# king159/Pair-Net

Hardware: AMD Instinct MI355X
Metric: images/sec (whole node), 100-query 800x1333, 1/2/4/8 MI355X (higher is better)
Workload: dtype f32

## Files before the change

### include/pairnet_hip.h

```cpp
#ifndef PAIRNET_HIP_H_
#define PAIRNET_HIP_H_

#include <stdint.h>

#ifdef __cplusplus
extern "C" {
#endif

#define PN_ABI_VERSION 34
int pn_abi_version(void);

#define PN_GEMM_RELU       1
#define PN_GEMM_A_COLMAJOR 2
#define PN_GEMM_FORCE_TILE 4
#define PN_GEMM_FORCE_SKINNY 8
#define PN_GEMM_FORCE_TILE64 16
#define PN_GEMM_FORCE_TILE128x64 32
#define PN_GEMM_RELU_AFTER_RES 128
#define PN_GEMM_GELU 256
#define PN_GEMM_RESERVE_SHIFT 16
#define PN_GEMM_RESERVE(n) ((((n) / 8) & 0x3ff) << PN_GEMM_RESERVE_SHIFT)
#define PN_GEMM_KSPLIT_SHIFT 26
#define PN_GEMM_KSPLIT(n) (((n) & 31) << PN_GEMM_KSPLIT_SHIFT)

// ... 442 lines not shown
typedef struct pn_gemm_s3_desc {
  const void* A;  const void* A2;  int32_t a2_from_col;
  const void* W;  const float* bias;
  int32_t M, N, K;
  int32_t relu;
  float* C;       int64_t ldc;
  void* CS;
  void* CS_pos;   const float* pos;  int32_t pos_rows;
  const void* res_s3;  const float* gamma;  const float* beta;  float eps;
  int32_t flags;
  int32_t act;  const float* res;  int64_t ldres;
} pn_gemm_s3_desc;
#define PN_GEMM_S3_TILE96 1
#define PN_GEMM_S3_TILE192 2
int pn_gemm_s3_f32(const pn_gemm_s3_desc* d, void* stream);

int pn_uniform_f32(float* out, int64_t n, int nsites, uint32_t site_stride, uint64_t seed,
                   uint32_t rank, uint32_t step, uint32_t site, void* stream);
int pn_seg_targets(const int64_t* table, const int32_t* row_ind, const int32_t* col_ind,
                   const int32_t* lsa_status, int nlsa, const int64_t* gt_labels, int64_t gt_len,
                   int64_t out_len, int L, int B, int Q, int C, int64_t Mtot, int64_t* labels,
                   int64_t* matched, int32_t* mcount, int32_t* status, void* stream);
int pn_uncertain_points_f32(const float* maps, int64_t nmaps, const int64_t* matched, int64_t M,
                            int B, int Q, int h, int w, const float* cand, const float* tail, int S,
                            int k, int Np, uint32_t* keys, float* pts, void* stream);
int pn_point_sample_rows_f32(const void* maps, int maps_are_u8, int64_t nmaps, const int64_t* idx,
                             const float* pts, float* out, int64_t M, int h, int w, int Np,
                             void* stream);
int pn_mask_point_loss_f32(const float* x, const float* t, const int64_t* matched, int64_t M, int Np,
                           int L, int Ml, float w_mask, float w_dice, float dice_eps,
// ... 80 lines not shown
```

### pair-net_amd/csrc/gemm_s3.hip

```cpp
#include "common.h"
#include "s3_common.h"

__device__ __forceinline__ void s3_glds16(const void* g, void* l) {
  __builtin_amdgcn_global_load_lds((const __attribute__((address_space(1))) void*)g,
                                   (__attribute__((address_space(3))) void*)l, 16, 0, 0);
}

__device__ __forceinline__ int64_t pos8_offset(int row, int col, int N) {
  return ((((int64_t)(row >> 5) * (N >> 4) + (col >> 4)) * 2 + ((col >> 3) & 1)) * 32 + (row & 31)) * 8;
}

__global__ __launch_bounds__(256) void k_s3_split(const float* __restrict__ X, int64_t ld,
                                                  const float* __restrict__ add, int add_rows,
                                                  uint4* __restrict__ S, int R, int K) {
  const int KB = K >> 4;
  const int lane = threadIdx.x & 63;
  const int64_t piece = (int64_t)blockIdx.x * 4 + (threadIdx.x >> 6);
  const int64_t npieces = (int64_t)((R + 31) >> 5) * KB;
  if (piece >= npieces) return;
  const int rb = (int)(piece / KB), kb = (int)(piece - (int64_t)rb * KB);
  const int r = rb * 32 + (lane & 31), k = kb * 16 + (lane >> 5) * 8;
  float v[8];
  if (r < R) {
    const float4 a = ld4(X + (int64_t)r * ld + k), b = ld4(X + (int64_t)r * ld + k + 4);
// ... 74 lines not shown
    }
    if (p.relu == 3) {
#pragma unroll
      for (int i = 0; i < 8; ++i) v[i] = fmaxf(v[i], 0.f);
    }
    if (p.C && row < p.M) {
      float* c = p.C + (int64_t)row * p.ldc + n0 + 16 * j + 8 * lh;
      st4(c, make_float4(v[0], v[1], v[2], v[3]));
      st4(c + 4, make_float4(v[4], v[5], v[6], v[7]));
    }
    if (p.CS) {
      s3_frag q0, q1, q2;
      s3_split8(v, q0, q1, q2);
      uint4* o = p.CS + ((int64_t)rb * KBo + (n0 >> 4) + j) * 192 + lane;
      o[0] = q0.u; o[64] = q1.u; o[128] = q2.u;
    }
  }
}

#ifndef S3_LATE_B
#define S3_LATE_B 0
#endif
template <bool LN>
__global__ __launch_bounds__(512, 1) void k_gemm_s3(const s3_args p) {
  constexpr int MB = 3, LATE_B = S3_LATE_B;
  constexpr int AH = 9 * 64, AST = 2 * AH;
  constexpr int BH = 24 * 64, BST = 2 * BH;
  constexpr int BRING = 3 * AST;
  __shared__ __attribute__((aligned(1024))) uint4 smem[3 * AST + 2 * BST];
  const int tid = threadIdx.x, lane = tid & 63, wave = __builtin_amdgcn_readfirstlane(tid >> 6);
// ... 129 lines not shown
      mma(s + 2 < S ? s + 2 : -1);
      if (s + 1 < S) drain_bar();
      as = as == 2 ? 0 : as + 1;
    }
  }

  const int n0 = tn * 256 + wave * 32;
  if (!LN) {
    if (n0 < N) {
#pragma unroll
      for (int m = 0; m < MB; ++m)
        if (rb0 + m < RB) s3_block_epilogue(acc[m], p, rb0 + m, n0, lane);
    }
    return;
  }
  const int li = lane & 31, lh = lane >> 5;
  const bool cols_ok = n0 < N;
  float v[MB][2][8];
#pragma unroll
  for (int m = 0; m < MB; ++m)
#pragma unroll
    for (int j = 0; j < 2; ++j)
#pragma unroll
      for (int i = 0; i < 4; ++i) {
        const auto sw = __builtin_amdgcn_permlane32_swap(__float_as_uint(acc[m][8 * j + i]),
                                                         __float_as_uint(acc[m][8 * j + 4 + i]), false, false);
        v[m][j][i] = __uint_as_float(sw[0]);
        v[m][j][4 + i] = __uint_as_float(sw[1]);
      }
  if (p.bias && cols_ok) {
#pragma unroll
    for (int j = 0; j < 2; ++j) {
      const float4 b0 = ld4(p.bias + n0 + 16 * j + 8 * lh), b1 = ld4(p.bias + n0 + 16 * j + 8 * lh + 4);
      const float bb[8] = {b0.x, b0.y, b0.z, b0.w, b1.x, b1.y, b1.z, b1.w};
#pragma unroll
      for (int m = 0; m < MB; ++m)
#pragma unroll
        for (int i = 0; i < 8; ++i) v[m][j][i] += bb[i];
    }
  }
  if (p.relu) {
#pragma unroll
    for (int m = 0; m < MB; ++m)
#pragma unroll
      for (int j = 0; j < 2; ++j)
#pragma unroll
        for (int i = 0; i < 8; ++i) v[m][j][i] = fmaxf(v[m][j][i], 0.f);
  }
  if (LN) {
#pragma clang fp contract(off)
    if (p.RES) {
#pragma unroll
      for (int m = 0; m < MB; ++m)
#pragma unroll
        for (int j = 0; j < 2; ++j) {
          const uint4* in = p.RES + ((int64_t)min(rb0 + m, RB - 1) * 16 + wave * 2 + j) * 192 + lane;
          s3_frag q0, q1, q2;
          q0.u = in[0]; q1.u = in[64]; q2.u = in[128];
          float r[8];
          s3_join8(q0, q1, q2, r);
#pragma unroll
          for (int i = 0; i < 8; ++i) v[m][j][i] += r[i];
        }
    }
    float* red = (float*)smem;
    __syncthreads();
    float s1[MB];
#pragma unroll
    for (int m = 0; m < MB; ++m) {
      float s = 0.f;
#pragma unroll
      for (int j = 0; j < 2; ++j)
#pragma unroll
        for (int i = 0; i < 8; ++i) s += v[m][j][i];
      s += __shfl_xor(s, 32, 64);
      if (lh == 0) red[wave * 96 + m * 32 + li] = s;
    }
    __syncthreads();
#pragma unroll
    for (int m = 0; m < MB; ++m) {
      float s = 0.f;
#pragma unroll
      for (int w = 0; w < 8; ++w) s += red[w * 96 + m * 32 + li];
      s1[m] = s * (1.f / 256.f);
    }
#pragma unroll
    for (int m = 0; m < MB; ++m) {
      float s = 0.f;
#pragma unroll
      for (int j = 0; j < 2; ++j)
#pragma unroll
        for (int i = 0; i < 8; ++i) { v[m][j][i] -= s1[m]; s += v[m][j][i] * v[m][j][i]; }
      s += __shfl_xor(s, 32, 64);
      if (lh == 0) red[768 + wave * 96 + m * 32 + li] = s;
    }
    __syncthreads();
    float g[2][8], be[2][8];
#pragma unroll
    for (int j = 0; j < 2; ++j) {
      const float4 g0 = ld4(p.gamma + n0 + 16 * j + 8 * lh), g1 = ld4(p.gamma + n0 + 16 * j + 8 * lh + 4);
      const float4 e0 = ld4(p.beta + n0 + 16 * j + 8 * lh), e1 = ld4(p.beta + n0 + 16 * j + 8 * lh + 4);
      g[j][0] = g0.x; g[j][1] = g0.y; g[j][2] = g0.z; g[j][3] = g0.w; g[j][4] = g1.x; g[j][5] = g1.y; g[j][6] = g1.z; g[j][7] = g1.w;
      be[j][0] = e0.x; be[j][1] = e0.y; be[j][2] = e0.z; be[j][3] = e0.w; be[j][4] = e1.x; be[j][5] = e1.y; be[j][6] = e1.z; be[j][7] = e1.w;
    }
#pragma unroll
    for (int m = 0; m < MB; ++m) {
      float s = 0.f;
#pragma unroll
      for (int w = 0; w < 8; ++w) s += red[768 + w * 96 + m * 32 + li];
      const float rstd = 1.f / sqrtf(s * (1.f / 256.f) + p.eps);
#pragma unroll
      for (int j = 0; j < 2; ++j)
#pragma unroll
        for (int i = 0; i < 8; ++i) v[m][j][i] = (v[m][j][i] * rstd) * g[j][i] + be[j][i];
    }
  }
  if (!cols_ok) return;
  const int KBo = p.nout >> 4;
#pragma unroll
  for (int m = 0; m < MB; ++m) {
    if (rb0 + m >= RB) break;
    const int row = (rb0 + m) * 32 + li;
#pragma unroll
    for (int j = 0; j < 2; ++j) {
      if (p.C && row < M) {
        float* c = p.C + (int64_t)row * p.ldc + n0 + 16 * j + 8 * lh;
        st4(c, make_float4(v[m][j][0], v[m][j][1], v[m][j][2], v[m][j][3]));
        st4(c + 4, make_float4(v[m][j][4], v[m][j][5], v[m][j][6], v[m][j][7]));
      }
      const int64_t piece = ((int64_t)(rb0 + m) * KBo + (n0 >> 4) + j) * 192 + lane;
      if (p.CS) {
        s3_frag q0, q1, q2;
        s3_split8(v[m][j], q0, q1, q2);
        uint4* o = p.CS + piece;
        o[0] = q0.u; o[64] = q1.u; o[128] = q2.u;
      }
      if (p.CSP) {
        const float* pp = p.pos + pos8_offset(min(row, M - 1) % p.pos_rows, n0 + 16 * j + 8 * lh, p.nout);
        const float4 p0 = ld4(pp), p1 = ld4(pp + 4);
        const float w[8] = {v[m][j][0] + p0.x, v[m][j][1] + p0.y, v[m][j][2] + p0.z, v[m][j][3] + p0.w,
                            v[m][j][4] + p1.x, v[m][j][5] + p1.y, v[m][j][6] + p1.z, v[m][j][7] + p1.w};
        s3_frag q0, q1, q2;
        s3_split8(w, q0, q1, q2);
        uint4* o = p.CSP + piece;
        o[0] = q0.u; o[64] = q1.u; o[128] = q2.u;
      }
    }
  }
}

__global__ __launch_bounds__(512, 1) void k_gemm_s3_wide(const s3_args p) {
  constexpr int MB = 3;
  constexpr int AS = 9 * 64, WS = 24 * 64;
  constexpr int WRING = 4 * AS;
  __shared__ __attribute__((aligned(1024))) uint4 smem[4 * AS + 3 * WS];
  const int tid = threadIdx.x, lane = tid & 63, wave = __builtin_amdgcn_readfirstlane(tid >> 6);
  const int grp = wave >> 2, wq = wave & 3;
  const int KB = p.K >> 4;
  const int RB = (p.M + 31) >> 5, CB = (p.N + 31) >> 5;
  const int nt = (p.N + 255) >> 8, mt = (RB + 2 * MB - 1) / (2 * MB);
  const int t = xcd_tile_index(blockIdx.x, nt * mt);
  const int tm = t / nt, tn = t - tm * nt;
  const int rb0 = tm * 2 * MB + grp * MB;
// ... 98 lines not shown
      if (j + 1 < KB) drain_bar();
      ws = ws == 2 ? 0 : ws + 1;
    }
  }
#pragma unroll
  for (int m = 0; m < MB; ++m) {
    if (rb0 + m >= RB) break;
#pragma unroll
    for (int c = 0; c < 2; ++c) {
      const int n0 = tn * 256 + wq * 64 + c * 32;
      if (n0 < p.N) s3_block_epilogue(acc[m][c], p, rb0 + m, n0, lane);
    }
  }
}

__global__ __launch_bounds__(256) void k_gemm_s3_narrow(const s3_args p, const int col0) {
  const int lane = threadIdx.x & 63;
  const int KB = p.K >> 4, RB = (p.M + 31) >> 5, ncb = (p.N - col0) >> 5;
  const int unit = blockIdx.x * 4 + (threadIdx.x >> 6);
  if (unit >= RB * ncb) return;
  const int rb = unit / ncb, cb = (col0 >> 5) + unit - rb * ncb;
  const uint4* ga = ((p.A2 && (cb >> 3) >= p.a2_from_tile) ? p.A2 : p.A) + (int64_t)rb * KB * 192 + lane;
  const uint4* gw = p.W + (int64_t)cb * KB * 192 + lane;
  f32x16 acc;
#pragma unroll
  for (int r = 0; r < 16; ++r) acc[r] = 0.f;
  constexpr int PA[6] = {2, 1, 0, 1, 0, 0}, PB[6] = {0, 1, 2, 0, 1, 0};
  constexpr int D = 4;
  s3_frag a[D][3], b[D][3];
  auto load = [&](int kb, int slot) {
// ... 22 lines not shown

extern "C" int pn_s3_split_f32(const float* X, int64_t ld, const float* add, int add_rows, void* S,
                               int rows, int K, void* stream) {
  if (!X || !S || rows <= 0 || K <= 0 || K % 16 || ld % 4 || (add && add_rows <= 0)) return PN_BAD_ARG;
  const int64_t np = (int64_t)((rows + 31) / 32) * (K / 16);
  k_s3_split<<<dim3((unsigned)((np + 3) / 4)), dim3(256), 0, (hipStream_t)stream>>>(
      X, ld, add, add ? add_rows : 1, (uint4*)S, rows, K);
  return PN_LAUNCH_CHECK();
}

extern "C" int pn_s3_join_f32(const void* S, float* X, int64_t ld, int rows, int K, void* stream) {
  if (!X || !S || rows <= 0 || K <= 0 || K % 16 || ld % 4) return PN_BAD_ARG;
  const int64_t np = (int64_t)((rows + 31) / 32) * (K / 16);
  k_s3_join<<<dim3((unsigned)((np + 3) / 4)), dim3(256), 0, (hipStream_t)stream>>>(
      (const uint4*)S, X, ld, rows, K);
  return PN_LAUNCH_CHECK();
}

extern "C" int pn_gemm_s3_f32(const pn_gemm_s3_desc* d, void* stream) {
  if (!d || !d->A || !d->W || d->M <= 0 || d->N <= 0 || d->K <= 0) return PN_BAD_ARG;
  if (d->K % 32 || d->N % 32) return PN_BAD_ARG;
  if (!d->C && !d->CS && !d->CS_pos) return PN_BAD_ARG;
  if (d->C && (d->ldc % 4 || d->ldc < d->N)) return PN_BAD_ARG;
  if (d->A2 && (d->a2_from_col <= 0 || d->a2_from_col % 256)) return PN_BAD_ARG;
  if (d->CS_pos && (!d->pos || d->pos_rows <= 0)) return PN_BAD_ARG;
  const bool ln = d->gamma != nullptr;
  if (ln && (d->N != 256 || !d->beta || d->relu)) return PN_BAD_ARG;
  if (!ln && d->res_s3) return PN_BAD_ARG;
  if (d->res && (ln || d->ldres % 4 || d->ldres < d->N)) return PN_BAD_ARG;
  if (d->act < 0 || d->act > 3 || (ln && d->act)) return PN_BAD_ARG;
// ... 47 lines not shown
```

### pair-net_amd/head.py

```python
import math
from collections import OrderedDict

import torch

from . import hip
from . import plans
from .plans import Arena, PlanCache, measure_bytes
from .config import ConfigDict

INSTANCE_OFFSET = 1000


def _decoder_param_shapes(prefix, num_layers, ffn_dim, out):
    for i in range(num_layers):
        p = "%s.layers.%d." % (prefix, i)
        for a in (0, 1):
            out[p + "attentions.%d.attn.in_proj_weight" % a] = (768, 256)
            out[p + "attentions.%d.attn.in_proj_bias" % a] = (768,)
            out[p + "attentions.%d.attn.out_proj.weight" % a] = (256, 256)
            out[p + "attentions.%d.attn.out_proj.bias" % a] = (256,)
        out[p + "ffns.0.layers.0.0.weight"] = (ffn_dim, 256)
        out[p + "ffns.0.layers.0.0.bias"] = (ffn_dim,)
        out[p + "ffns.0.layers.1.weight"] = (256, ffn_dim)
        out[p + "ffns.0.layers.1.bias"] = (256,)
# ... 87 lines not shown
        self.device = None
        self.w = None
        self._plans = PlanCache()
        self._arenas, self._post_arenas, self._consts, self._pe = {}, {}, {}, OrderedDict()
        self._dummies = {}
        self._post = OrderedDict()
        self._pan_jobs = []
        self.graph_after = 1
        self.exact_mask_order = True
        self.conv_algo = "winograd4"
        self.use_graphs = False
        self.grid_reserve = 0
        self.fuse_ppn_front = True
        self.fuse_mask_pack = True
        self.gather_mask_stencil = True
        self.fuse_lateral_upadd = False
        self.enc_fused_ln = ("proj", "ffn")
        self.group_input_convs = False
        self.gemm_arithmetic = "bf16x3"
        self.msda_s3_out = False
        self.fused_pair_masks = True
        self.init_weights()

    def param_shapes(self):
        s = OrderedDict()
        Q, R = self.num_obj_query, self.num_rel_query
        _decoder_param_shapes("relation_decoder", self.num_rel_layers, self.rel_ffn, s)
        s["rel_query_embed.weight"] = (R, 256)
        s["rel_query_embed2.weight"] = (2 * R, 256)
        s["rel_query_embed3.weight"] = (2 * R, 256)
# ... 499 lines not shown
            if "ffn" in self.enc_fused_ln:
                hip.linear_res_ln(pl.H, w[p + "ffns.0.layers.1.weight"],
                                  w[p + "ffns.0.layers.1.bias"], X12, w[p + "norms.1.weight"],
                                  w[p + "norms.1.bias"], X2)
            else:
                hip.linear(pl.H, w[p + "ffns.0.layers.1.weight"], w[p + "ffns.0.layers.1.bias"],
                           Y2, res=X12)
                hip.layernorm(Y2, w[p + "norms.1.weight"], w[p + "norms.1.bias"], X2)

    def _encoder_s3(self, pl):
        w, B, SN = self.w, pl.B, pl.SN
        pd = "pixel_decoder."
        M, F = B * SN, self.enc_ffn
        X2 = pl.X.view(-1, 256)
        pos8 = (pl.enc_pos8, SN)
        hip.s3_split(X2, pl.XS)
        hip.s3_split(X2, pl.XPS, add=pl.enc_pos)
        for i in range(self.num_enc_layers):
            p = pd + "encoder.layers.%d." % i
            a = p + "attentions.0."
            last = i + 1 == self.num_enc_layers
            hip.gemm_s3(pl.XS, w[a + "voa.weight.s3"], M, 544, 256, bias=w[a + "voa.bias"],
                        out=pl.VOA.view(-1, 544), a2=pl.XPS, a2_from_col=256)
            if self.msda_s3_out:
                hip.msda(pl.VOA, 544, pl.VOA.view(-1)[256:], 544, pl.SS, B, pl.shapes, s3_out=True)
            else:
                hip.msda(pl.VOA, 544, pl.VOA.view(-1)[256:], 544, pl.S, B, pl.shapes)
                hip.s3_split(pl.S.view(-1, 256), pl.SS)
            hip.gemm_s3(pl.SS, w[a + "output_proj.weight.s3"], M, 256, 256,
                        bias=w[a + "output_proj.bias"], out_s3=pl.X1S, res_s3=pl.XS,
                        gamma=w[p + "norms.0.weight"], beta=w[p + "norms.0.bias"])
            hip.gemm_s3(pl.X1S, w[p + "ffns.0.layers.0.0.weight.s3"], M, F, 256,
                        bias=w[p + "ffns.0.layers.0.0.bias"], relu=True, out_s3=pl.HS)
            hip.gemm_s3(pl.HS, w[p + "ffns.0.layers.1.weight.s3"], M, 256, F,
                        bias=w[p + "ffns.0.layers.1.bias"], res_s3=pl.X1S,
                        gamma=w[p + "norms.1.weight"], beta=w[p + "norms.1.bias"],
                        out=X2 if last else None, out_s3=None if last else pl.XS,
                        out_s3_pos=None if last else pl.XPS, pos=pos8)

    def _mlp3(self, prefix, src, dst, pl):
        w = self.w
        hip.linear(src, w[prefix + ".0.weight"], w[prefix + ".0.bias"], pl.m1, relu=True)
        hip.linear(pl.m1, w[prefix + ".2.weight"], w[prefix + ".2.bias"], pl.m2, relu=True)
        hip.linear(pl.m2, w[prefix + ".4.weight"], w[prefix + ".4.bias"], dst)

    def _mask_logits(self, me, pl, out):
        Q = self.num_obj_query
        hip.gemm(me, pl.MF, out, M=Q, N=pl.HW2, K=256, lda=256, ldw=256, ldc=pl.HW2,
                 batch=pl.B, sA=Q * 256, sW=pl.HW2 * 256, sC=Q * pl.HW2)

    def _head_embed(self, q, pl, with_cls, full_mask, cls_out=None, mp_out=None, normed=False):
        w, B, Q = self.w, pl.B, self.num_obj_query
        cls_out = pl.cls if cls_out is None else cls_out
# ... 207 lines not shown
        for f, c in zip(feats, self.in_channels):
            if not f.is_cuda or f.dtype != torch.float32 or f.shape[1] != c or not (nchw or nhwc):
                raise RuntimeError("feats must be fp32 [B,C,H,W] device tensors with channels %s, "
                                   "all contiguous or all in channels_last memory format"
                                   % self.in_channels)
        if self.device is None:
            self.to(feats[0].device)
        shapes = [tuple(feats[3 - l].shape[-2:]) for l in range(3)]
        self._feats_nhwc = nhwc
        return B, shapes, tuple(feats[0].shape[-2:])

    def _run_stage(self, which, pl, feats=None):
        cfg = (self.exact_mask_order, self.conv_algo, self.fuse_ppn_front, self.grid_reserve,
               tuple(self.enc_fused_ln), self.group_input_convs,
               getattr(self, "fuse_mask_pack", True), self.gemm_arithmetic, self.msda_s3_out,
               self._fused_pair_masks(),
               getattr(self, "gather_mask_stencil", True), getattr(self, "fuse_lateral_upadd", False))
        if pl.graph_cfg != cfg:
            pl.graph_a = pl.graph_b = None
            pl.graphs_a = OrderedDict()
            pl.graph_c = PlanCache(self.POST_VIEWS)
            pl.graph_cfg = cfg
        cur = torch.cuda.current_stream(self.device)
        pl.streams[cur.cuda_stream] = cur
        try:
            self._run_stage_on(which, pl, feats, cur)
        finally:
            plans.note_use(cur)

    def _run_stage_on(self, which, pl, feats, cur):
        if which == "a":
# ... 349 lines not shown
```

### pair-net_amd/hip.py

```python
import contextlib
import ctypes as C
import os
import threading

import torch

from .build import LIB_PATH

LIB_PATH = os.environ.get("PAIRNET_LIB") or LIB_PATH

_i32, _i64, _f32, _vp = C.c_int32, C.c_int64, C.c_float, C.c_void_p

GEMM_RELU, GEMM_A_COLMAJOR, GEMM_FORCE_TILE, GEMM_FORCE_SKINNY = 1, 2, 4, 8
GEMM_GELU = 256
GEMM_FORCE_TILE64, GEMM_FORCE_TILE128x64 = 16, 32
GEMM_RELU_AFTER_RES = 128
GEMM_GROUP_MAX = 18


class GemmDesc(C.Structure):
    _fields_ = [("A", _vp), ("lda", _i64), ("strideA", _i64),
                ("Aadd", _vp), ("ldaadd", _i64), ("aadd_rows", _i32),
                ("aadd_from_col", _i32),
                ("W", _vp), ("ldw", _i64), ("strideW", _i64),
# ... 4 lines not shown
                ("flags", _i32),
                ("splitk_scratch", _vp), ("splitk_scratch_floats", _i64)]


class GemmS3Desc(C.Structure):
    _fields_ = [("A", _vp), ("A2", _vp), ("a2_from_col", _i32),
                ("W", _vp), ("bias", _vp),
                ("M", _i32), ("N", _i32), ("K", _i32), ("relu", _i32),
                ("C", _vp), ("ldc", _i64),
                ("CS", _vp),
                ("CS_pos", _vp), ("pos", _vp), ("pos_rows", _i32),
                ("res_s3", _vp), ("gamma", _vp), ("beta", _vp), ("eps", _f32), ("flags", _i32),
                ("act", _i32), ("res", _vp), ("ldres", _i64)]


_SIGS = {
    "pn_abi_version": (C.c_int, []),
    "pn_s3_bytes": (_i64, [_i32, _i32]),
    "pn_s3_split_f32": (C.c_int, [_vp, _i64, _vp, _i32, _vp, _i32, _i32, _vp]),
    "pn_s3_join_f32": (C.c_int, [_vp, _vp, _i64, _i32, _i32, _vp]),
    "pn_gemm_s3_f32": (C.c_int, [C.POINTER(GemmS3Desc), _vp]),
    "pn_gemm_f32": (C.c_int, [C.POINTER(GemmDesc), _vp]),
    "pn_gemm_variant": (C.c_int, [C.POINTER(GemmDesc)]),
    "pn_gemm_grid_size": (C.c_int, [C.POINTER(GemmDesc)]),
    "pn_gemm_wgs_per_cu": (C.c_int, []),
    "pn_gemm_group_f32": (C.c_int, [C.POINTER(GemmDesc), C.c_int, _vp]),
    "pn_conv2d_nhwc_f32": (C.c_int, [_vp, _vp, _vp, _vp] + [_i32] * 10 + [_vp]),
    "pn_conv2d_nhwc_ex_f32": (C.c_int, [_vp] * 5 + [_i32] * 10 + [_vp, _i64, _vp]),
    "pn_bottleneck_proj_f32": (C.c_int, [_vp] * 8 + [_i32] * 8 + [_vp, _i64, _vp]),
    "pn_stem7x7s2_f32": (C.c_int, [_vp, _vp, _vp, _vp, _i32, _i32, _i32, _i32, _vp]),
    "pn_maxpool3x3s2_nhwc_f32": (C.c_int, [_vp, _vp, _i32, _i32, _i32, _i32, _vp]),
    "pn_winograd_f23_input_f32": (C.c_int, [_vp, _vp, _i32, _i32, _i32, _i32, _vp]),
    "pn_winograd_f23_output_f32": (C.c_int, [_vp, _vp, _vp, _i32, _i32, _i32, _i32, _i32, _vp]),
    "pn_winograd_f43_input_f32": (C.c_int, [_vp, _vp, _i32, _i32, _i32, _i32, _vp]),
    "pn_winograd_f43_output_f32": (C.c_int, [_vp, _vp, _vp, _i32, _i32, _i32, _i32, _i32, _vp]),
    "pn_layernorm_f32": (C.c_int, [_vp, _vp, _vp, _vp, _i64, _i32, _f32, _vp]),
# ... 605 lines not shown
        d.pos, d.pos_rows = _ptr(pos), pr
    d.res_s3, d.gamma, d.beta, d.eps = _ptr(res_s3), _ptr(gamma), _ptr(beta), eps
    d.flags = (1 if tile96 else 0) | (2 if tile192 else 0)
    d.act = 3 if relu_after else 2 if gelu else 0
    if res is not None:
        Mr, ldr = _rowmajor(res)
        assert Mr == M and res.shape[1] >= N
        d.res, d.ldres = _ptr(res), ldr
    nbytes = 6.0 * (M * K + N * K) + (4.0 * M * N if out is not None else 0.0) + \
        6.0 * M * N * ((out_s3 is not None) + (out_s3_pos is not None) + (res_s3 is not None))
    name = "k_gemm_s3<ln>" if gamma is not None else "k_gemm_s3"
    _check(_launch(name, 2.0 * M * N * K, nbytes, lambda: lib().pn_gemm_s3_f32(C.byref(d), _stream()),
                   meta=(M, N, K, 1, False)), "pn_gemm_s3_f32")


def layernorm_rows(x, gamma, beta, out, eps=1e-5):
    rows, ldx = _rowmajor(x)
    ro, ldo = _rowmajor(out)
    assert ro == rows and out.shape[1] == x.shape[1]
    _check(_launch("k_ln_rows", 0.0, 8.0 * rows * x.shape[1],
                   lambda: lib().pn_layernorm_rows_f32(_ptr(x), ldx, _ptr(gamma), _ptr(beta),
                                                       _ptr(out), ldo, rows, x.shape[1], eps,
                                                       _stream())), "pn_layernorm_rows_f32")


def layernorm_rows_s3(x, gamma, beta, out_s3, eps=1e-5):
    rows, ldx = _rowmajor(x)
    Cc = x.shape[1]
    assert out_s3.numel() >= s3_floats(rows, Cc)
    _check(_launch("k_ln_rows<s3>", 0.0, 10.0 * rows * Cc,
# ... 1319 lines not shown
```

Before: 229.4.

## Fuse encoder FFN into one kernel keeping hidden activations on-chip

Adds a k_gemm_s3_ffn kernel that computes the encoder FFN (GEMM1 + bias + ReLU, then GEMM2 + bias + residual + LayerNorm) in a single launch. The hidden activation is produced in 256-wide chunks, split into s3 pieces and written straight into shared memory for the second GEMM. This avoids writing and re-reading the large hidden tensor HS through global memory, and saves one launch per layer. The LN epilogue is factored into a shared helper. In exchange, each workgroup recomputes over the whole F dimension with a fixed 3-row-block tile and a complex wave-specialised schedule, so parallelism is limited to M/96 workgroups, which risks underfilling the GPU.

```diff
diff --git a/include/pairnet_hip.h b/include/pairnet_hip.h
--- a/include/pairnet_hip.h
+++ b/include/pairnet_hip.h
@@ -480,6 +480,17 @@
 #define PN_GEMM_S3_TILE96 1
 #define PN_GEMM_S3_TILE192 2
 int pn_gemm_s3_f32(const pn_gemm_s3_desc* d, void* stream);
+typedef struct pn_gemm_s3_ffn_desc {
+  const void* X;  const void* W1;  const float* b1;
+  const void* W2; const float* b2;
+  int32_t M, N, K, F;
+  int32_t act;
+  float* C;       int64_t ldc;
+  void* CS;
+  void* CS_pos;   const float* pos;  int32_t pos_rows;
+  const void* res_s3;  const float* gamma;  const float* beta;  float eps;
+} pn_gemm_s3_ffn_desc;
+int pn_gemm_s3_ffn_f32(const pn_gemm_s3_ffn_desc* d, void* stream);
 
 int pn_uniform_f32(float* out, int64_t n, int nsites, uint32_t site_stride, uint64_t seed,
                    uint32_t rank, uint32_t step, uint32_t site, void* stream);
diff --git a/pair-net_amd/csrc/gemm_s3.hip b/pair-net_amd/csrc/gemm_s3.hip
--- a/pair-net_amd/csrc/gemm_s3.hip
+++ b/pair-net_amd/csrc/gemm_s3.hip
@@ -112,6 +112,145 @@
       s3_split8(v, q0, q1, q2);
       uint4* o = p.CS + ((int64_t)rb * KBo + (n0 >> 4) + j) * 192 + lane;
       o[0] = q0.u; o[64] = q1.u; o[128] = q2.u;
+    }
+  }
+}
+
+__device__ __forceinline__ void s3_ln_epilogue(const f32x16 (&acc)[3], const s3_args& p, uint4* smem,
+                                               int rb0, int n0, int wave, int lane) {
+  constexpr int MB = 3;
+  const int M = p.M, RB = (M + 31) >> 5;
+  const int li = lane & 31, lh = lane >> 5;
+  const bool cols_ok = n0 < p.N;
+  float v[MB][2][8];
+#pragma unroll
+  for (int m = 0; m < MB; ++m)
+#pragma unroll
+    for (int j = 0; j < 2; ++j)
+#pragma unroll
+      for (int i = 0; i < 4; ++i) {
+        const auto sw = __builtin_amdgcn_permlane32_swap(__float_as_uint(acc[m][8 * j + i]),
+                                                         __float_as_uint(acc[m][8 * j + 4 + i]), false, false);
+        v[m][j][i] = __uint_as_float(sw[0]);
+        v[m][j][4 + i] = __uint_as_float(sw[1]);
+      }
+  if (p.bias && cols_ok) {
+#pragma unroll
+    for (int j = 0; j < 2; ++j) {
+      const float4 b0 = ld4(p.bias + n0 + 16 * j + 8 * lh), b1 = ld4(p.bias + n0 + 16 * j + 8 * lh + 4);
+      const float bb[8] = {b0.x, b0.y, b0.z, b0.w, b1.x, b1.y, b1.z, b1.w};
+#pragma unroll
+      for (int m = 0; m < MB; ++m)
+#pragma unroll
+        for (int i = 0; i < 8; ++i) v[m][j][i] += bb[i];
+    }
+  }
+  if (p.relu) {
+#pragma unroll
+    for (int m = 0; m < MB; ++m)
+#pragma unroll
+      for (int j = 0; j < 2; ++j)
+#pragma unroll
+        for (int i = 0; i < 8; ++i) v[m][j][i] = fmaxf(v[m][j][i], 0.f);
+  }
+  {
+#pragma clang fp contract(off)
+    if (p.RES) {
+#pragma unroll
+      for (int m = 0; m < MB; ++m)
+#pragma unroll
+        for (int j = 0; j < 2; ++j) {
+          const uint4* in = p.RES + ((int64_t)min(rb0 + m, RB - 1) * 16 + wave * 2 + j) * 192 + lane;
+          s3_frag q0, q1, q2;
+          q0.u = in[0]; q1.u = in[64]; q2.u = in[128];
+          float r[8];
+          s3_join8(q0, q1, q2, r);
+#pragma unroll
+          for (int i = 0; i < 8; ++i) v[m][j][i] += r[i];
+        }
+    }
+    float* red = (float*)smem;
+    __syncthreads();
+    float s1[MB];
+#pragma unroll
+    for (int m = 0; m < MB; ++m) {
+      float s = 0.f;
+#pragma unroll
+      for (int j = 0; j < 2; ++j)
+#pragma unroll
+        for (int i = 0; i < 8; ++i) s += v[m][j][i];
+      s += __shfl_xor(s, 32, 64);
+      if (lh == 0) red[wave * 96 + m * 32 + li] = s;
+    }
+    __syncthreads();
+#pragma unroll
+    for (int m = 0; m < MB; ++m) {
+      float s = 0.f;
+#pragma unroll
+      for (int w = 0; w < 8; ++w) s += red[w * 96 + m * 32 + li];
+      s1[m] = s * (1.f / 256.f);
+    }
+#pragma unroll
+    for (int m = 0; m < MB; ++m) {
+      float s = 0.f;
+#pragma unroll
+      for (int j = 0; j < 2; ++j)
+#pragma unroll
+        for (int i = 0; i < 8; ++i) { v[m][j][i] -= s1[m]; s += v[m][j][i] * v[m][j][i]; }
+      s += __shfl_xor(s, 32, 64);
+      if (lh == 0) red[768 + wave * 96 + m * 32 + li] = s;
+    }
+    __syncthreads();
+    float g[2][8], be[2][8];
+#pragma unroll
+    for (int j = 0; j < 2; ++j) {
+      const float4 g0 = ld4(p.gamma + n0 + 16 * j + 8 * lh), g1 = ld4(p.gamma + n0 + 16 * j + 8 * lh + 4);
+      const float4 e0 = ld4(p.beta + n0 + 16 * j + 8 * lh), e1 = ld4(p.beta + n0 + 16 * j + 8 * lh + 4);
+      g[j][0] = g0.x; g[j][1] = g0.y; g[j][2] = g0.z; g[j][3] = g0.w; g[j][4] = g1.x; g[j][5] = g1.y; g[j][6] = g1.z; g[j][7] = g1.w;
+      be[j][0] = e0.x; be[j][1] = e0.y; be[j][2] = e0.z; be[j][3] = e0.w; be[j][4] = e1.x; be[j][5] = e1.y; be[j][6] = e1.z; be[j][7] = e1.w;
+    }
+#pragma unroll
+    for (int m = 0; m < MB; ++m) {
+      float s = 0.f;
+#pragma unroll
+      for (int w = 0; w < 8; ++w) s += red[768 + w * 96 + m * 32 + li];
+      const float rstd = 1.f / sqrtf(s * (1.f / 256.f) + p.eps);
+#pragma unroll
+      for (int j = 0; j < 2; ++j)
+#pragma unroll
+        for (int i = 0; i < 8; ++i) v[m][j][i] = (v[m][j][i] * rstd) * g[j][i] + be[j][i];
+    }
+  }
+  if (!cols_ok) return;
+  const int KBo = p.nout >> 4;
+#pragma unroll
+  for (int m = 0; m < MB; ++m) {
+    if (rb0 + m >= RB) break;
+    const int row = (rb0 + m) * 32 + li;
+#pragma unroll
+    for (int j = 0; j < 2; ++j) {
+      if (p.C && row < M) {
+        float* c = p.C + (int64_t)row * p.ldc + n0 + 16 * j + 8 * lh;
+        st4(c, make_float4(v[m][j][0], v[m][j][1], v[m][j][2], v[m][j][3]));
+        st4(c + 4, make_float4(v[m][j][4], v[m][j][5], v[m][j][6], v[m][j][7]));
+      }
+      const int64_t piece = ((int64_t)(rb0 + m) * KBo + (n0 >> 4) + j) * 192 + lane;
+      if (p.CS) {
+        s3_frag q0, q1, q2;
+        s3_split8(v[m][j], q0, q1, q2);
+        uint4* o = p.CS + piece;
+        o[0] = q0.u; o[64] = q1.u; o[128] = q2.u;
+      }
+      if (p.CSP) {
+        const float* pp = p.pos + pos8_offset(min(row, M - 1) % p.pos_rows, n0 + 16 * j + 8 * lh, p.nout);
+        const float4 p0 = ld4(pp), p1 = ld4(pp + 4);
+        const float w[8] = {v[m][j][0] + p0.x, v[m][j][1] + p0.y, v[m][j][2] + p0.z, v[m][j][3] + p0.w,
+                            v[m][j][4] + p1.x, v[m][j][5] + p1.y, v[m][j][6] + p1.z, v[m][j][7] + p1.w};
+        s3_frag q0, q1, q2;
+        s3_split8(w, q0, q1, q2);
+        uint4* o = p.CSP + piece;
+        o[0] = q0.u; o[64] = q1.u; o[128] = q2.u;
+      }
     }
   }
 }
@@ -271,139 +410,7 @@
     }
     return;
   }
-  const int li = lane & 31, lh = lane >> 5;
-  const bool cols_ok = n0 < N;
-  float v[MB][2][8];
-#pragma unroll
-  for (int m = 0; m < MB; ++m)
-#pragma unroll
-    for (int j = 0; j < 2; ++j)
-#pragma unroll
-      for (int i = 0; i < 4; ++i) {
-        const auto sw = __builtin_amdgcn_permlane32_swap(__float_as_uint(acc[m][8 * j + i]),
-                                                         __float_as_uint(acc[m][8 * j + 4 + i]), false, false);
-        v[m][j][i] = __uint_as_float(sw[0]);
-        v[m][j][4 + i] = __uint_as_float(sw[1]);
-      }
-  if (p.bias && cols_ok) {
-#pragma unroll
-    for (int j = 0; j < 2; ++j) {
-      const float4 b0 = ld4(p.bias + n0 + 16 * j + 8 * lh), b1 = ld4(p.bias + n0 + 16 * j + 8 * lh + 4);
-      const float bb[8] = {b0.x, b0.y, b0.z, b0.w, b1.x, b1.y, b1.z, b1.w};
-#pragma unroll
-      for (int m = 0; m < MB; ++m)
-#pragma unroll
-        for (int i = 0; i < 8; ++i) v[m][j][i] += bb[i];
-    }
-  }
-  if (p.relu) {
-#pragma unroll
-    for (int m = 0; m < MB; ++m)
-#pragma unroll
-      for (int j = 0; j < 2; ++j)
-#pragma unroll
-        for (int i = 0; i < 8; ++i) v[m][j][i] = fmaxf(v[m][j][i], 0.f);
-  }
-  if (LN) {
-#pragma clang fp contract(off)
-    if (p.RES) {
-#pragma unroll
-      for (int m = 0; m < MB; ++m)
-#pragma unroll
-        for (int j = 0; j < 2; ++j) {
-          const uint4* in = p.RES + ((int64_t)min(rb0 + m, RB - 1) * 16 + wave * 2 + j) * 192 + lane;
-          s3_frag q0, q1, q2;
-          q0.u = in[0]; q1.u = in[64]; q2.u = in[128];
-          float r[8];
-          s3_join8(q0, q1, q2, r);
-#pragma unroll
-          for (int i = 0; i < 8; ++i) v[m][j][i] += r[i];
-        }
-    }
-    float* red = (float*)smem;
-    __syncthreads();
-    float s1[MB];
-#pragma unroll
-    for (int m = 0; m < MB; ++m) {
-      float s = 0.f;
-#pragma unroll
-      for (int j = 0; j < 2; ++j)
-#pragma unroll
-        for (int i = 0; i < 8; ++i) s += v[m][j][i];
-      s += __shfl_xor(s, 32, 64);
-      if (lh == 0) red[wave * 96 + m * 32 + li] = s;
-    }
-    __syncthreads();
-#pragma unroll
-    for (int m = 0; m < MB; ++m) {
-      float s = 0.f;
-#pragma unroll
-      for (int w = 0; w < 8; ++w) s += red[w * 96 + m * 32 + li];
-      s1[m] = s * (1.f / 256.f);
-    }
-#pragma unroll
-    for (int m = 0; m < MB; ++m) {
-      float s = 0.f;
-#pragma unroll
-      for (int j = 0; j < 2; ++j)
-#pragma unroll
-        for (int i = 0; i < 8; ++i) { v[m][j][i] -= s1[m]; s += v[m][j][i] * v[m][j][i]; }
-      s += __shfl_xor(s, 32, 64);
-      if (lh == 0) red[768 + wave * 96 + m * 32 + li] = s;
-    }
-    __syncthreads();
-    float g[2][8], be[2][8];
-#pragma unroll
-    for (int j = 0; j < 2; ++j) {
-      const float4 g0 = ld4(p.gamma + n0 + 16 * j + 8 * lh), g1 = ld4(p.gamma + n0 + 16 * j + 8 * lh + 4);
-      const float4 e0 = ld4(p.beta + n0 + 16 * j + 8 * lh), e1 = ld4(p.beta + n0 + 16 * j + 8 * lh + 4);
-      g[j][0] = g0.x; g[j][1] = g0.y; g[j][2] = g0.z; g[j][3] = g0.w; g[j][4] = g1.x; g[j][5] = g1.y; g[j][6] = g1.z; g[j][7] = g1.w;
-      be[j][0] = e0.x; be[j][1] = e0.y; be[j][2] = e0.z; be[j][3] = e0.w; be[j][4] = e1.x; be[j][5] = e1.y; be[j][6] = e1.z; be[j][7] = e1.w;
-    }
-#pragma unroll
-    for (int m = 0; m < MB; ++m) {
-      float s = 0.f;
-#pragma unroll
-      for (int w = 0; w < 8; ++w) s += red[768 + w * 96 + m * 32 + li];
-      const float rstd = 1.f / sqrtf(s * (1.f / 256.f) + p.eps);
-#pragma unroll
-      for (int j = 0; j < 2; ++j)
-#pragma unroll
-        for (int i = 0; i < 8; ++i) v[m][j][i] = (v[m][j][i] * rstd) * g[j][i] + be[j][i];
-    }
-  }
-  if (!cols_ok) return;
-  const int KBo = p.nout >> 4;
-#pragma unroll
-  for (int m = 0; m < MB; ++m) {
-    if (rb0 + m >= RB) break;
-    const int row = (rb0 + m) * 32 + li;
-#pragma unroll
-    for (int j = 0; j < 2; ++j) {
-      if (p.C && row < M) {
-        float* c = p.C + (int64_t)row * p.ldc + n0 + 16 * j + 8 * lh;
-        st4(c, make_float4(v[m][j][0], v[m][j][1], v[m][j][2], v[m][j][3]));
-        st4(c + 4, make_float4(v[m][j][4], v[m][j][5], v[m][j][6], v[m][j][7]));
-      }
-      const int64_t piece = ((int64_t)(rb0 + m) * KBo + (n0 >> 4) + j) * 192 + lane;
-      if (p.CS) {
-        s3_frag q0, q1, q2;
-        s3_split8(v[m][j], q0, q1, q2);
-        uint4* o = p.CS + piece;
-        o[0] = q0.u; o[64] = q1.u; o[128] = q2.u;
-      }
-      if (p.CSP) {
-        const float* pp = p.pos + pos8_offset(min(row, M - 1) % p.pos_rows, n0 + 16 * j + 8 * lh, p.nout);
-        const float4 p0 = ld4(pp), p1 = ld4(pp + 4);
-        const float w[8] = {v[m][j][0] + p0.x, v[m][j][1] + p0.y, v[m][j][2] + p0.z, v[m][j][3] + p0.w,
-                            v[m][j][4] + p1.x, v[m][j][5] + p1.y, v[m][j][6] + p1.z, v[m][j][7] + p1.w};
-        s3_frag q0, q1, q2;
-        s3_split8(w, q0, q1, q2);
-        uint4* o = p.CSP + piece;
-        o[0] = q0.u; o[64] = q1.u; o[128] = q2.u;
-      }
-    }
-  }
+  s3_ln_epilogue(acc, p, smem, rb0, n0, wave, lane);
 }
 
 __global__ __launch_bounds__(512, 1) void k_gemm_s3_wide(const s3_args p) {
@@ -532,6 +539,217 @@
   }
 }
 
+__global__ __launch_bounds__(512, 1) void k_gemm_s3_ffn(const s3_args p, const uint4* __restrict__ W1,
+                                                        const float* __restrict__ b1) {
+  constexpr int MB = 3;
+  constexpr int AH = 9 * 64, AST = 2 * AH;
+  constexpr int BH = 24 * 64, BST = 2 * BH;
+  constexpr int BRING = 3 * AST;
+  constexpr int CHUNK1 = 8 * 16 * 192;
+  __shared__ __attribute__((aligned(1024))) uint4 smem[3 * AST + 2 * BST];
+  const int tid = threadIdx.x, lane = tid & 63, wave = __builtin_amdgcn_readfirstlane(tid >> 6);
+  const int grp = wave >> 2, wq = wave & 3;
+  const int M = p.M, KB2 = p.K >> 4, NC = p.K >> 8;
+  const int RB = (M + 31) >> 5, mt = (RB + MB - 1) / MB;
+  const int rb0 = xcd_tile_index(blockIdx.x, mt) * MB;
+
+  const int cb = grp * 4 + wq;
+  const uint4* gW1 = W1 + cb * 16 * 192;
+  const uint4* gW2 = p.W + (int64_t)cb * KB2 * 192;
+  const uint4* gX = p.A + (int64_t)min(rb0 + wq, RB - 1) * 16 * 192;
+  const int lW = cb * 3 * 64, lX = wq * 3 * 64;
+  const bool xw = wq < 3;
+  const unsigned ul = lane;
+  auto issueW1 = [&](int c, int u) {
+    const uint4* g = gW1 + (int64_t)c * CHUNK1 + u * 384;
+    const int base = BRING + (u & 1) * BST + lW;
+#pragma unroll
+    for (int h = 0; h < 2; ++h)
+#pragma unroll
+      for (int q = 0; q < 3; ++q) s3_glds16(g + (h * 192 + q * 64) + ul, &smem[base + h * BH + q * 64]);
+  };
+  auto issueW2 = [&](int c, int s) {
+    const uint4* g = gW2 + (c * 8 + s) * 384;
+    const int base = BRING + (s & 1) * BST + lW;
+#pragma unroll
+    for (int h = 0; h < 2; ++h)
+#pragma unroll
+      for (int q = 0; q < 3; ++q) s3_glds16(g + (h * 192 + q * 64) + ul, &smem[base + h * BH + q * 64]);
+  };
+  auto issueA = [&](int u, int as, int half) {
+    if (!xw) return;
+    const uint4* g = gX + (2 * u + half) * 192;
+    const int base = as * AST + half * AH + lX;
+#pragma unroll
+    for (int q = 0; q < 3; ++q) s3_glds16(g + q * 64 + ul, &smem[base + q * 64]);
+  };
+  s3_frag a[2][MB][3], b[2][3];
+  const int bfrag = (grp * 4 + wq) * 3 * 64 + lane;
+  auto read = [&](int ws, int as) {
+    const uint4* pa = smem + as * AST + lane;
+    const uint4* pb = smem + BRING + ws * BST + bfrag;
+#pragma unroll
+    for (int h = 0; h < 2; ++h) {
+#pragma unroll
+      for (int m = 0; m < MB; ++m)
+#pragma unroll
+        for (int q = 0; q < 3; ++q) a[h][m][q].u = pa[h * AH + (m * 3 + q) * 64];
+#pragma unroll
+      for (int q = 0; q < 3; ++q) b[h][q].u = pb[h * BH + q * 64];
+    }
+  };
+  auto mma = [&](f32x16 (&acc)[MB]) {
+    constexpr int PA[6] = {2, 1, 0, 1, 0, 0}, PB[6] = {0, 1, 2, 0, 1, 0};
+#pragma unroll
+    for (int h = 0; h < 2; ++h)
+#pragma unroll
+      for (int q = 0; q < 6; ++q)
+#pragma unroll
+        for (int m = 0; m < MB; ++m)
+          acc[m] = __builtin_amdgcn_mfma_f32_32x32x16_bf16(b[h][PB[q]].v, a[h][m][PA[q]].v, acc[m], 0, 0, 0);
+  };
+  auto bar = [&] {
+    __builtin_amdgcn_sched_barrier(0);
+    asm volatile("" ::: "memory");
+    __builtin_amdgcn_s_barrier();
+    asm volatile("" ::: "memory");
+    __builtin_amdgcn_sched_barrier(0);
+  };
+  auto drain_bar = [&] {
+    __builtin_amdgcn_sched_barrier(0);
+    __builtin_amdgcn_s_waitcnt(0x0070);
+    bar();
+  };
+  f32x16 acc1[MB], acc2[MB];
+#pragma unroll
+  for (int m = 0; m < MB; ++m)
+#pragma unroll
+    for (int r = 0; r < 16; ++r) acc2[m][r] = 0.f;
+  s3_frag pc[MB][2][3];
+  auto make_pieces = [&](int c) {
+    const int lh = lane >> 5;
+#pragma unroll
+    for (int m = 0; m < MB; ++m) {
+#pragma unroll
+      for (int j = 0; j < 2; ++j) {
+        float v[8];
+#pragma unroll
+        for (int i = 0; i < 4; ++i) {
+          const auto sw = __builtin_amdgcn_permlane32_swap(__float_as_uint(acc1[m][8 * j + i]),
+                                                           __float_as_uint(acc1[m][8 * j + 4 + i]), false, false);
+          v[i] = __uint_as_float(sw[0]);
+          v[4 + i] = __uint_as_float(sw[1]);
+        }
+        if (b1) {
+          const float* bp = b1 + c * 256 + wave * 32 + 16 * j + 8 * lh;
+          const float4 b0 = ld4(bp), b1v = ld4(bp + 4);
+          v[0] += b0.x; v[1] += b0.y; v[2] += b0.z; v[3] += b0.w; v[4] += b1v.x; v[5] += b1v.y; v[6] += b1v.z; v[7] += b1v.w;
+        }
+#pragma unroll
+        for (int i = 0; i < 8; ++i) v[i] = fmaxf(v[i], 0.f);
+        s3_split8(v, pc[m][j][0], pc[m][j][1], pc[m][j][2]);
+#pragma unroll
+        for (int q = 0; q < 3; ++q)
+          asm volatile("" : "+v"(pc[m][j][q].u.x), "+v"(pc[m][j][q].u.y), "+v"(pc[m][j][q].u.z), "+v"(pc[m][j][q].u.w));
+      }
+    }
+  };
+  auto write_pieces = [&](int as) {
+    uint4* d = smem + as * AST + lane;
+#pragma unroll
+    for (int j = 0; j < 2; ++j)
+#pragma unroll
+      for (int m = 0; m < MB; ++m)
+#pragma unroll
+        for (int q = 0; q < 3; ++q) d[j * AH + (m * 3 + q) * 64] = pc[m][j][q].u;
+  };
+  auto zero1 = [&] {
+#pragma unroll
+    for (int m = 0; m < MB; ++m)
+#pragma unroll
+      for (int r = 0; r < 16; ++r) acc1[m][r] = 0.f;
+  };
+
+  issueW1(0, 0);
+  issueA(0, 0, grp);
+  if (grp == 1) issueA(1, 1, 1);
+  drain_bar();
+  int as = 0;
+  if (grp == 0) {
+    for (int c = 0; c < NC; ++c) {
+      zero1();
+#pragma unroll 1
+      for (int u = 0; u < 8; ++u) {
+        const int as1 = as == 2 ? 0 : as + 1;
+        __builtin_amdgcn_s_setprio(1);
+        read(u & 1, as);
+        if (u < 7) { issueW1(c, u + 1); issueA(u + 1, as1, 0); }
+        else issueW2(c, 0);
+        __builtin_amdgcn_s_setprio(0);
+        bar();
+        mma(acc1);
+        drain_bar();
+        as = as1;
+      }
+      make_pieces(c);
+      if (wave < 2) write_pieces(wave == 0 ? as : (as == 2 ? 0 : as + 1));
+      drain_bar();
+#pragma unroll 1
+      for (int s = 0; s < 8; ++s) {
+        const int as1 = as == 2 ? 0 : as + 1;
+        __builtin_amdgcn_s_setprio(1);
+        read(s & 1, as);
+        if (s < 7) issueW2(c, s + 1);
+        else if (c + 1 < NC) { issueW1(c + 1, 0); issueA(0, as1, 0); }
+        __builtin_amdgcn_s_setprio(0);
+        bar();
+        mma(acc2);
+        if (wave == s + 2) write_pieces(as == 0 ? 2 : as - 1);
+        drain_bar();
+        as = as1;
+      }
+    }
+  } else {
+    bar();
+    for (int c = 0; c < NC; ++c) {
+      zero1();
+#pragma unroll 1
+      for (int u = 0; u < 8; ++u) {
+        const int as2 = as == 0 ? 2 : as - 1;
+        __builtin_amdgcn_s_setprio(1);
+        read(u & 1, as);
+        if (u < 7) issueW1(c, u + 1);
+        else issueW2(c, 0);
+        if (u + 2 < 8) issueA(u + 2, as2, 1);
+        __builtin_amdgcn_s_setprio(0);
+        bar();
+        mma(acc1);
+        drain_bar();
+        as = as == 2 ? 0 : as + 1;
+      }
+      make_pieces(c);
+      bar();
+#pragma unroll 1
+      for (int s = 0; s < 8; ++s) {
+        const int as2 = as == 0 ? 2 : as - 1;
+        const bool more = c + 1 < NC;
+        __builtin_amdgcn_s_setprio(1);
+        read(s & 1, as);
+        if (s < 7) issueW2(c, s + 1);
+        else if (more) issueW1(c + 1, 0);
+        if (s >= 6 && more) issueA(s - 6, as2, 1);
+        __builtin_amdgcn_s_setprio(0);
+        bar();
+        mma(acc2);
+        if (wave == s + 2) write_pieces(as2);
+        if (more || s < 7) drain_bar();
+        as = as == 2 ? 0 : as + 1;
+      }
+    }
+  }
+  s3_ln_epilogue(acc2, p, smem, rb0, wave * 32, wave, lane);
+}
+
 __global__ __launch_bounds__(256) void k_gemm_s3_narrow(const s3_args p, const int col0) {
   const int lane = threadIdx.x & 63;
   const int KB = p.K >> 4, RB = (p.M + 31) >> 5, ncb = (p.N - col0) >> 5;
@@ -584,6 +802,27 @@
   const int64_t np = (int64_t)((rows + 31) / 32) * (K / 16);
   k_s3_join<<<dim3((unsigned)((np + 3) / 4)), dim3(256), 0, (hipStream_t)stream>>>(
       (const uint4*)S, X, ld, rows, K);
+  return PN_LAUNCH_CHECK();
+}
+
+extern "C" int pn_gemm_s3_ffn_f32(const pn_gemm_s3_ffn_desc* d, void* stream) {
+  if (!d || !d->X || !d->W1 || !d->W2 || d->M <= 0) return PN_BAD_ARG;
+  if (d->K != 256 || d->N != 256 || d->F <= 0 || d->F % 256) return PN_BAD_ARG;
+  if (d->act != 1) return PN_BAD_ARG;
+  if (!d->gamma || !d->beta) return PN_BAD_ARG;
+  if (!d->C && !d->CS && !d->CS_pos) return PN_BAD_ARG;
+  if (d->C && (d->ldc % 4 || d->ldc < d->N)) return PN_BAD_ARG;
+  if (d->CS_pos && (!d->pos || d->pos_rows <= 0)) return PN_BAD_ARG;
+  s3_args a;
+  a.A = (const uint4*)d->X; a.A2 = nullptr; a.a2_from_tile = 0;
+  a.W = (const uint4*)d->W2; a.bias = d->b2;
+  a.C = d->C; a.ldc = d->ldc; a.CS = (uint4*)d->CS; a.CSP = (uint4*)d->CS_pos;
+  a.RES = (const uint4*)d->res_s3; a.gamma = d->gamma; a.beta = d->beta; a.pos = d->pos;
+  a.pos_rows = d->pos_rows; a.eps = d->eps;
+  a.M = d->M; a.N = d->N; a.K = d->F; a.relu = 0; a.nout = d->N;
+  a.res = nullptr; a.ldres = 0;
+  const int RB = (d->M + 31) / 32, mt = (RB + 2) / 3;
+  k_gemm_s3_ffn<<<dim3(mt), dim3(512), 0, (hipStream_t)stream>>>(a, (const uint4*)d->W1, d->b1);
   return PN_LAUNCH_CHECK();
 }
 
diff --git a/pair-net_amd/head.py b/pair-net_amd/head.py
--- a/pair-net_amd/head.py
+++ b/pair-net_amd/head.py
@@ -125,6 +125,7 @@
         self.fuse_ppn_front = True
         self.fuse_mask_pack = True
         self.gather_mask_stencil = True
+        self.fuse_encoder_ffn = 1
         self.fuse_lateral_upadd = False
         self.enc_fused_ln = ("proj", "ffn")
         self.group_input_convs = False
@@ -654,6 +655,7 @@
         M, F = B * SN, self.enc_ffn
         X2 = pl.X.view(-1, 256)
         pos8 = (pl.enc_pos8, SN)
+        fuse_ffn = bool(getattr(self, "fuse_encoder_ffn", 0)) and F % 256 == 0
         hip.s3_split(X2, pl.XS)
         hip.s3_split(X2, pl.XPS, add=pl.enc_pos)
         for i in range(self.num_enc_layers):
@@ -670,13 +672,19 @@
             hip.gemm_s3(pl.SS, w[a + "output_proj.weight.s3"], M, 256, 256,
                         bias=w[a + "output_proj.bias"], out_s3=pl.X1S, res_s3=pl.XS,
                         gamma=w[p + "norms.0.weight"], beta=w[p + "norms.0.bias"])
+            tail = dict(res_s3=pl.X1S, gamma=w[p + "norms.1.weight"], beta=w[p + "norms.1.bias"],
+                        out=X2 if last else None, out_s3=None if last else pl.XS,
+                        out_s3_pos=None if last else pl.XPS, pos=pos8)
+            if fuse_ffn:
+                hip.gemm_s3_ffn(pl.X1S, w[p + "ffns.0.layers.0.0.weight.s3"],
+                                w[p + "ffns.0.layers.1.weight.s3"], M, 256, 256, F,
+                                b1=w[p + "ffns.0.layers.0.0.bias"],
+                                b2=w[p + "ffns.0.layers.1.bias"], **tail)
+                continue
             hip.gemm_s3(pl.X1S, w[p + "ffns.0.layers.0.0.weight.s3"], M, F, 256,
                         bias=w[p + "ffns.0.layers.0.0.bias"], relu=True, out_s3=pl.HS)
             hip.gemm_s3(pl.HS, w[p + "ffns.0.layers.1.weight.s3"], M, 256, F,
-                        bias=w[p + "ffns.0.layers.1.bias"], res_s3=pl.X1S,
-                        gamma=w[p + "norms.1.weight"], beta=w[p + "norms.1.bias"],
-                        out=X2 if last else None, out_s3=None if last else pl.XS,
-                        out_s3_pos=None if last else pl.XPS, pos=pos8)
+                        bias=w[p + "ffns.0.layers.1.bias"], **tail)
 
     def _mlp3(self, prefix, src, dst, pl):
         w = self.w
@@ -914,7 +922,7 @@
         cfg = (self.exact_mask_order, self.conv_algo, self.fuse_ppn_front, self.grid_reserve,
                tuple(self.enc_fused_ln), self.group_input_convs,
                getattr(self, "fuse_mask_pack", True), self.gemm_arithmetic, self.msda_s3_out,
-               self._fused_pair_masks(),
+               self._fused_pair_masks(), bool(getattr(self, "fuse_encoder_ffn", 0)),
                getattr(self, "gather_mask_stencil", True), getattr(self, "fuse_lateral_upadd", False))
         if pl.graph_cfg != cfg:
             pl.graph_a = pl.graph_b = None
diff --git a/pair-net_amd/hip.py b/pair-net_amd/hip.py
--- a/pair-net_amd/hip.py
+++ b/pair-net_amd/hip.py
@@ -42,12 +42,22 @@
                 ("act", _i32), ("res", _vp), ("ldres", _i64)]
 
 
+class GemmS3FfnDesc(C.Structure):
+    _fields_ = [("X", _vp), ("W1", _vp), ("b1", _vp), ("W2", _vp), ("b2", _vp),
+                ("M", _i32), ("N", _i32), ("K", _i32), ("F", _i32), ("act", _i32),
+                ("C", _vp), ("ldc", _i64),
+                ("CS", _vp),
+                ("CS_pos", _vp), ("pos", _vp), ("pos_rows", _i32),
+                ("res_s3", _vp), ("gamma", _vp), ("beta", _vp), ("eps", _f32)]
+
+
 _SIGS = {
     "pn_abi_version": (C.c_int, []),
     "pn_s3_bytes": (_i64, [_i32, _i32]),
     "pn_s3_split_f32": (C.c_int, [_vp, _i64, _vp, _i32, _vp, _i32, _i32, _vp]),
     "pn_s3_join_f32": (C.c_int, [_vp, _vp, _i64, _i32, _i32, _vp]),
     "pn_gemm_s3_f32": (C.c_int, [C.POINTER(GemmS3Desc), _vp]),
+    "pn_gemm_s3_ffn_f32": (C.c_int, [C.POINTER(GemmS3FfnDesc), _vp]),
     "pn_gemm_f32": (C.c_int, [C.POINTER(GemmDesc), _vp]),
     "pn_gemm_variant": (C.c_int, [C.POINTER(GemmDesc)]),
     "pn_gemm_grid_size": (C.c_int, [C.POINTER(GemmDesc)]),
@@ -683,6 +693,28 @@
                    meta=(M, N, K, 1, False)), "pn_gemm_s3_f32")
 
 
+def gemm_s3_ffn(x, w1, w2, M, N, K, F, *, b1=None, b2=None, res_s3=None, gamma=None, beta=None,
+                eps=1e-5, out=None, out_s3=None, out_s3_pos=None, pos=None, gelu=False):
+    d = GemmS3FfnDesc()
+    d.X, d.W1, d.b1, d.W2, d.b2 = _ptr(x), _ptr(w1), _ptr(b1), _ptr(w2), _ptr(b2)
+    d.M, d.N, d.K, d.F, d.act = M, N, K, F, 2 if gelu else 1
+    if out is not None:
+        Mo, ldc = _rowmajor(out)
+        assert Mo == M and out.shape[1] >= N
+        d.C, d.ldc = _ptr(out), ldc
+    d.CS, d.CS_pos = _ptr(out_s3), _ptr(out_s3_pos)
+    if out_s3_pos is not None:
+        pos, pr = pos
+        assert pos.numel() == (pr + 31) // 32 * 32 * N
+        d.pos, d.pos_rows = _ptr(pos), pr
+    d.res_s3, d.gamma, d.beta, d.eps = _ptr(res_s3), _ptr(gamma), _ptr(beta), eps
+    nbytes = 6.0 * (M * K + 2 * F * K) + (4.0 * M * N if out is not None else 0.0) + \
+        6.0 * M * N * ((out_s3 is not None) + (out_s3_pos is not None) + (res_s3 is not None))
+    _check(_launch("k_gemm_s3_ffn", 2.0 * M * F * (K + N), nbytes,
+                   lambda: lib().pn_gemm_s3_ffn_f32(C.byref(d), _stream()),
+                   meta=(M, N, F, 1, False)), "pn_gemm_s3_ffn_f32")
+
+
 def layernorm_rows(x, gamma, beta, out, eps=1e-5):
     rows, ldx = _rowmajor(x)
     ro, ldo = _rowmajor(out)
```

New measurement: 233.7 (median of 6 runs). +1.9%, better.
